# laclouis5/StructureDetector

Hardware: NVIDIA B200
Metric: decoded images/s (higher is better)
Workload: dtype f32

## Files before the change

### structuredetector_b200/csrc/common.cuh

```cuda
#pragma once

#include <cuda.h>
#include <cuda_bf16.h>
#include <cuda_fp16.h>
#include <cuda_runtime.h>
#include <math_constants.h>
#include <stdint.h>
#include <stdlib.h>

#include "sdnet_decode.h"

namespace {

typedef unsigned long long u64;
typedef unsigned int u32;

constexpr int kThreads = 256;
constexpr int kWarps = kThreads / 32;
constexpr int kPanelW = 128;
constexpr int kBins = 128;
constexpr float kBinLo = -16.0f;
constexpr float kBinScale = 4.0f;
constexpr int kFineBins = 512;
constexpr float kFineScale = 16.0f;
// ... 52 lines not shown
    const float s = __half2float(__float2half_rn(1.0f / (1.0f + expf(-x))));
    return __half2float(__float2half_rn(fminf(fmaxf(s, kClampLo), kClampHi)));
  }
  static __device__ __forceinline__ float to_float(__half v) { return __half2float(v); }
};

template <>
struct Num<SDNET_DTYPE_BF16> {
  typedef __nv_bfloat16 In;
  static constexpr float kNear = 0.1f, kHi = 2.0f, kLo = -13.0f;
  static constexpr float kNear2 = 0.6f, kHi2 = 4.0f;
  static __device__ __forceinline__ float act(float x) {
    const float s = __bfloat162float(__float2bfloat16_rn(1.0f / (1.0f + expf(-x))));
    return __bfloat162float(__float2bfloat16_rn(fminf(fmaxf(s, kClampLo), kClampHi)));
  }
  static __device__ __forceinline__ float to_float(__nv_bfloat16 v) { return __bfloat162float(v); }
};

template <int DT>
__device__ __forceinline__ float ld_in(const void* base, long long idx) {
  return Num<DT>::to_float(__ldg(static_cast<const typename Num<DT>::In*>(base) + idx));
}

__device__ __forceinline__ float max3(float a, float b, float c) { return fmaxf(fmaxf(a, b), c); }

__device__ __forceinline__ void pdl_launch_dependents() { asm volatile("griddepcontrol.launch_dependents;" ::: "memory"); }
__device__ __forceinline__ void pdl_wait() { asm volatile("griddepcontrol.wait;" ::: "memory"); }

__device__ __forceinline__ float comp(const float4& v, int j) {
  return j == 0 ? v.x : (j == 1 ? v.y : (j == 2 ? v.z : v.w));
}

__device__ __forceinline__ u32 smem_u32(const void* p) { return (u32)__cvta_generic_to_shared(p); }
__device__ __forceinline__ void cp_async4_if(u32 dst, const void* src, bool pred) {
  asm volatile("{\n\t.reg .pred p;\n\tsetp.ne.b32 p, %2, 0;\n\t@p cp.async.ca.shared.global [%0], [%1], 4;\n\t}"
               ::"r"(dst), "l"(src), "r"((int)pred));
}
__device__ __forceinline__ void cp_async_commit() { asm volatile("cp.async.commit_group;" ::: "memory"); }
template <int N>
__device__ __forceinline__ void cp_async_wait() { asm volatile("cp.async.wait_group %0;" ::"n"(N) : "memory"); }
__device__ __forceinline__ float4 lds128(u32 addr) {
  float4 v;
  asm volatile("ld.shared.v4.f32 {%0, %1, %2, %3}, [%4];" : "=f"(v.x), "=f"(v.y), "=f"(v.z), "=f"(v.w) : "r"(addr));
  return v;
}
__device__ __forceinline__ float2 lds64(u32 addr) {
  float2 v;
  asm volatile("ld.shared.v2.f32 {%0, %1}, [%2];" : "=f"(v.x), "=f"(v.y) : "r"(addr));
  return v;
}
__device__ __forceinline__ void sts128(u32 addr, float a) {
  asm volatile("st.shared.v4.f32 [%0], {%1, %1, %1, %1};" ::"r"(addr), "f"(a) : "memory");
}
__device__ __forceinline__ void sts64(u32 addr, float a) {
  asm volatile("st.shared.v2.f32 [%0], {%1, %1};" ::"r"(addr), "f"(a) : "memory");
}

__device__ __forceinline__ void mbar_init(u32 bar, u32 count) {
  asm volatile("mbarrier.init.shared::cta.b64 [%0], %1;" ::"r"(bar), "r"(count) : "memory");
}
__device__ __forceinline__ void mbar_fence_init() { asm volatile("fence.mbarrier_init.release.cluster;" ::: "memory"); }
__device__ __forceinline__ void mbar_arrive_expect_tx(u32 bar, u32 bytes) {
  asm volatile("mbarrier.arrive.expect_tx.shared::cta.b64 _, [%0], %1;" ::"r"(bar), "r"(bytes) : "memory");
}
#ifndef SDNET_X_WAIT_NS
#define SDNET_X_WAIT_NS 1000
#endif
__device__ __forceinline__ void mbar_wait(u32 bar, u32 parity) {
#if SDNET_X_WAIT_NS > 0
  asm volatile(
      "{\n\t.reg .pred p;\n"
      "WAIT_LOOP:\n\t"
      "mbarrier.try_wait.parity.shared::cta.b64 p, [%0], %1, %2;\n\t"
      "@!p bra WAIT_LOOP;\n\t}"
      ::"r"(bar), "r"(parity), "r"((u32)SDNET_X_WAIT_NS) : "memory");
#else
  asm volatile(
      "{\n\t.reg .pred p;\n"
      "WAIT_LOOP:\n\t"
      "mbarrier.try_wait.parity.shared::cta.b64 p, [%0], %1;\n\t"
      "@!p bra WAIT_LOOP;\n\t}"
      ::"r"(bar), "r"(parity) : "memory");
#endif
}
__device__ __forceinline__ void fence_proxy_async() { asm volatile("fence.proxy.async.shared::cta;" ::: "memory"); }

}
```

### structuredetector_b200/csrc/floors.cuh

```cuda
#pragma once

namespace {

#ifndef SDNET_X_BUF
#define SDNET_X_BUF 64
#endif
constexpr int kBuf = SDNET_X_BUF;
#ifndef SDNET_X_GRATE
#define SDNET_X_GRATE 0
#endif
#ifndef SDNET_X_LRATE
#define SDNET_X_LRATE 0
#endif
constexpr int kGRate = SDNET_X_GRATE, kLRate = SDNET_X_LRATE;
constexpr int kGDiv = kGRate ? kGRate : 1, kLDiv = kLRate ? kLRate : 1;

__device__ __forceinline__ int logit_bin(float x) {
  int bin = __float2int_rd((x - kBinLo) * kBinScale);
  bin = max(0, min(kBins - 1, bin));
  if (bin > 0 && x < kBinLo + (float)bin * (1.0f / kBinScale)) --bin;
  return bin;
}

__device__ __forceinline__ int ord_of(float x) {
  const int b = __float_as_int(x);
  return b ^ ((b >> 31) & 0x7fffffff);
}
__device__ __forceinline__ float ord_to_float(int o) { return __int_as_float(o ^ ((o >> 31) & 0x7fffffff)); }

__device__ __forceinline__ int floor_bin_of(const uint4 c, int lane, int K) {
  const u32 s = c.x + c.y + c.z + c.w;
  u32 suf = s;
#pragma unroll
  for (int d = 1; d < 32; d <<= 1) {
    u32 t = __shfl_down_sync(0xffffffffu, suf, d);
    if (lane + d < 32) suf += t;
  }
  const u32 mask = __ballot_sync(0xffffffffu, suf >= (u32)K);
  if (mask == 0) return -1;
  const int L = 31 - __clz(mask);
  int b = 0;
  if (lane == L) {
    u32 above = suf - s;
    if (above + c.w >= (u32)K) b = 4 * L + 3;
    else if (above + c.w + c.z >= (u32)K) b = 4 * L + 2;
    else if (above + c.w + c.z + c.y >= (u32)K) b = 4 * L + 1;
    else b = 4 * L;
  }
  return __shfl_sync(0xffffffffu, b, L);
}

__device__ __forceinline__ float local_floor(const u32* hist, const int* minx, int lane, int K) {
  const int b = floor_bin_of(*reinterpret_cast<const uint4*>(hist + 4 * lane), lane, K);
  if (b < 0) return -CUDART_INF_F;
  return ord_to_float(minx[b]);
}

__device__ __forceinline__ int fine_bin(float x) {
  static_assert(kBinLo == -16.0f && kFineScale == 16.0f, "bin arithmetic below");
  return max(0, min(kFineBins - 1, __float2int_rd(fminf(fmaxf(x * kFineScale, -4096.0f), 4096.0f)) + 256));
// ... 16 lines not shown
  uint4 v[kFinePerLane / 4];
#pragma unroll
  for (int q = 0; q < kFinePerLane / 4; ++q) v[q] = load_bins<kShared>(mine + 4 * q);
  u32 s = 0;
#pragma unroll
  for (int q = 0; q < kFinePerLane / 4; ++q) s += v[q].x + v[q].y + v[q].z + v[q].w;
  u32 suf = s;
#pragma unroll
  for (int d = 1; d < 32; d <<= 1) {
    u32 t = __shfl_down_sync(0xffffffffu, suf, d);
    if (lane + d < 32) suf += t;
  }
  const u32 mask = __ballot_sync(0xffffffffu, suf >= (u32)K);
  if (mask == 0) return -1;
  const int L = 31 - __clz(mask);
  int b = kFinePerLane * L;
  if (lane == L) {
    u32 above = suf - s;
    bool found = false;
#pragma unroll
    for (int q = kFinePerLane / 4 - 1; q >= 0; --q) {
      const u32 c4[4] = {v[q].x, v[q].y, v[q].z, v[q].w};
#pragma unroll
      for (int e = 3; e >= 0; --e) {
        if (!found) {
          if (above + c4[e] >= (u32)K) { b = kFinePerLane * L + 4 * q + e; found = true; }
          else above += c4[e];
        }
      }
    }
  }
  return __shfl_sync(0xffffffffu, b, L);
}

template <int DT = SDNET_DTYPE_F32>
__device__ __forceinline__ float shared_floor(int fbin, float xscale) {
  const bool pre = xscale != 1.0f;
  if (fbin <= 0) return pre ? 0.0f : -CUDART_INF_F;
  const float edge = kBinLo + (float)fbin * (1.0f / kFineScale);
  if (pre) return fmaxf(edge / xscale, 0.0f);
  if (edge < Num<DT>::kLo || edge > Num<DT>::kHi2) return -CUDART_INF_F;
  return edge - (edge <= Num<DT>::kHi ? Num<DT>::kNear : Num<DT>::kNear2);
}

struct SharedFloors {
  u32* ghist;
  int* gfloor;
};

struct UnitState {
  float floorx;
  u32 emitted;
  int nbuf;
};

template <int DT = SDNET_DTYPE_F32, bool kFlushCountsFine = true>
__device__ __forceinline__ void flush_candidates(UnitState& st, const u64* buf, u32* hist, int* minx,
                                                 const SharedFloors& sf, int* count_ptr, u64* __restrict__ list,
                                                 int cap, int K, int lane, bool pre, float xscale, float satx) {
  const int n = st.nbuf;
  int base = 0;
  if (lane == 0) base = atomicAdd(count_ptr, n);
  base = __shfl_sync(0xffffffffu, base, 0);
#pragma unroll
  for (int half = 0; half < kBuf / 32; ++half) {
    const int i = half * 32 + lane;
    if (half * 32 < n) {
      const bool valid = i < n;
      const u64 rec = valid ? buf[i] : 0ull;
      const float x = __uint_as_float((u32)(rec >> 32));
      u32 key;
      if (pre) {
        const u32 bits = __float_as_uint(x);
        key = (bits & 0x80000000u) ? ~bits : (bits | 0x80000000u);
      } else {
        key = __float_as_uint(Num<DT>::act(x));
      }
      if (valid) {
        if (base + i < cap) list[base + i] = ((u64)key << 32) | (u32)rec;
        const float xe = fminf(fmaxf(x * xscale, -satx), satx);
        const int bin = logit_bin(xe);
        atomicAdd(&hist[bin], 1u);
        atomicMin(&minx[bin], ord_of(xe));
        if (kFlushCountsFine && sf.ghist) atomicAdd(&sf.ghist[fine_bin(xe)], 1u);
      }
    }
  }
  const u32 before = st.emitted;
  st.emitted += n;
  st.nbuf = 0;
  __syncwarp();
  if (st.emitted >= (u32)K && (kLRate == 0 || before < (u32)K || before / kLDiv != st.emitted / kLDiv))
    st.floorx = fmaxf(st.floorx, local_floor(hist, minx, lane, K) / xscale);
  if (sf.ghist && base + n >= K && (kGRate == 0 || base < K || base / kGDiv != (base + n) / kGDiv)) {
    const int gb = floor_bin_fine<false>(sf.ghist, lane, K);
    if (gb > 0) {
      if (lane == 0) atomicMax(sf.gfloor, gb);
      st.floorx = fmaxf(st.floorx, shared_floor<DT>(gb, xscale));
    }
  }
  if (st.floorx >= satx) st.floorx = CUDART_INF_F;
}


}
```

### structuredetector_b200/csrc/peaks_tile.cuh

```cuda
#pragma once

namespace {

constexpr int kGroupRows = 4;
constexpr int kTileCols = kPanelW + 8;
constexpr int kTilePitchB = kTileCols * 4;
constexpr int kTileBytes = kGroupRows * kTilePitchB;
#ifndef SDNET_X_WARPS
#define SDNET_X_WARPS 4
#endif
constexpr int kTileWarps = SDNET_X_WARPS;
#ifndef SDNET_X_CTAS
#define SDNET_X_CTAS (24 / SDNET_X_WARPS)
#endif
constexpr int kTileMinCtas = SDNET_X_CTAS;
constexpr int kMinChunkGroups = 8;
#ifndef SDNET_X_NG
#define SDNET_X_NG 3
#endif
constexpr int kTileNG = SDNET_X_NG;
#ifndef SDNET_X_FLUSH_AT
#define SDNET_X_FLUSH_AT 16
#endif
constexpr int kWork = 128;
constexpr int kFlushAt = SDNET_X_FLUSH_AT;
__host__ __device__ constexpr int tile_slot_bytes(int S) { return S == 1 ? kTileBytes : 2304; }
__host__ __device__ constexpr int tile_smem_per_warp(int S) {
  return ((kTileNG * tile_slot_bytes(S) + 32 + kBins * 8 + kBuf * 8 + kWork) + 127) / 128 * 128;
}
__host__ __device__ constexpr int tile_smem(int S) { return kTileWarps * tile_smem_per_warp(S); }
constexpr int kOddBoxOff = 1152;
constexpr int kOddShiftB = 8;

template <int DT>
struct TileGeom {
  static constexpr int kPx = DT == SDNET_DTYPE_F32 ? 4 : 8;
  static constexpr int kEsz = 16 / kPx;
  static constexpr int kPanel = 32 * kPx;
  static constexpr int kCols = kPanel + 2 * kPx;
};
static_assert(TileGeom<SDNET_DTYPE_F32>::kCols * 4 == kTilePitchB && TileGeom<SDNET_DTYPE_F16>::kCols * 2 == kTilePitchB, "ring row pitch");

__device__ __forceinline__ void tma_tile_4d(u32 dst, const CUtensorMap* map, int x, int y, int c, int b, u32 bar) {
  asm volatile(
      "cp.async.bulk.tensor.4d.shared::cluster.global.tile.mbarrier::complete_tx::bytes [%0], [%1, {%2, %3, %4, %5}], [%6];"
      ::"r"(dst), "l"(map), "r"(x), "r"(y), "r"(c), "r"(b), "r"(bar) : "memory");
}
__device__ __forceinline__ uint4 lds64x2(u32 addr) {
  uint4 v;
  asm volatile("ld.shared.v2.u32 {%0, %1}, [%2];" : "=r"(v.x), "=r"(v.y) : "r"(addr));
  asm volatile("ld.shared.v2.u32 {%0, %1}, [%2];" : "=r"(v.z), "=r"(v.w) : "r"(addr + 8));
  return v;
}
__device__ __forceinline__ uint4 lds128u(u32 addr) {
  uint4 v;
  asm volatile("ld.shared.v4.u32 {%0, %1, %2, %3}, [%4];" : "=r"(v.x), "=r"(v.y), "=r"(v.z), "=r"(v.w) : "r"(addr));
  return v;
}

template <int DT>
struct TileMax;
template <>
struct TileMax<SDNET_DTYPE_F32> {
  static __device__ __forceinline__ float word(const uint4& a) {
    return fmaxf(fmaxf(__uint_as_float(a.x), __uint_as_float(a.y)), fmaxf(__uint_as_float(a.z), __uint_as_float(a.w)));
  }
  static __device__ __forceinline__ float group(const uint4& a, const uint4& b, const uint4& c, const uint4& d) {
    return fmaxf(fmaxf(word(a), word(b)), fmaxf(word(c), word(d)));
  }
  static __device__ __forceinline__ float elem(u32 addr) {
    float v;
    asm volatile("ld.shared.f32 %0, [%1];" : "=f"(v) : "r"(addr));
    return v;
  }
  static __device__ __forceinline__ u32 raw(u32 addr) { return __float_as_uint(elem(addr)); }
  static __device__ __forceinline__ u32 rmax(u32 a, u32 b) { return __float_as_uint(fmaxf(__uint_as_float(a), __uint_as_float(b))); }
  static __device__ __forceinline__ float rfloat(u32 r) { return __uint_as_float(r); }
};
template <>
struct TileMax<SDNET_DTYPE_F16> {
  static __device__ __forceinline__ __half2 h2(u32 v) { return *reinterpret_cast<const __half2*>(&v); }
  static __device__ __forceinline__ __half2 word2(const uint4& a) { return __hmax2(__hmax2(h2(a.x), h2(a.y)), __hmax2(h2(a.z), h2(a.w))); }
  static __device__ __forceinline__ float fold(__half2 m) { return __half2float(__hmax(__low2half(m), __high2half(m))); }
// ... 84 lines not shown
    for (int d = 0; d <= 2 * R; ++d) {
      u32 rr = row0 + i + d;
      if (rr >= kRingRows) rr -= kRingRows;
      roff[d] = S == 1 ? rr * kTilePitchB : __shfl_sync(0xffffffffu, row_tab, (int)rr);
    }
    const float x = TileMax<DT>::elem(col_addr + R * kEsz + roff[R]);
    bool keep = slot < nslots && x > floorx;
#if SDNET_X_QUICK
    if (!pre) {
      const u32 ctr = col_addr + R * kEsz;
      const float m4 = fmaxf(fmaxf(TileMax<DT>::elem(ctr + roff[R - 1]), TileMax<DT>::elem(ctr + roff[R + 1])),
                             fmaxf(TileMax<DT>::elem(ctr - kEsz + roff[R]), TileMax<DT>::elem(ctr + kEsz + roff[R])));
      if (x < m4 - kNearTie2 && x <= kHiZone2 - 1.0f && x >= kLoZone) keep = false;
    }
#endif
    if (keep && !pre) {
      u32 hr[2 * R + 1];
#pragma unroll
      for (int d = 0; d <= 2 * R; ++d) {
        const u32 a = col_addr + roff[d];
        u32 v[2 * R + 1];
#pragma unroll
        for (int q = 0; q <= 2 * R; ++q) v[q] = TileMax<DT>::raw(a + kEsz * q);
        hr[d] = v[0];
#pragma unroll
        for (int q = 1; q <= 2 * R; ++q) hr[d] = TileMax<DT>::rmax(hr[d], v[q]);
      }
#pragma unroll
      for (int d = 1; d <= 2 * R; ++d) hr[0] = TileMax<DT>::rmax(hr[0], hr[d]);
      const float h = fmaxf(x, TileMax<DT>::rfloat(hr[0]));
      if (x != h) {
        const bool amb = (x >= h - kNearTie) || (h > kHiZone && x >= h - kNearTie2) ||
                         (h > kHiZone2 && x > kHiZone2 - 1.0f) || (h < kLoZone);
        keep = amb && Num<DT>::act(x) == Num<DT>::act(h);
      }
    }
    const u32 m = __ballot_sync(0xffffffffu, keep);
    if (m) {
      if (st.nbuf + __popc(m) > kBuf) {
        __syncwarp();
        flush_candidates<DT, !SDNET_X_EARLYHIST>(st, buf, hist, minx, sf, count_ptr, list, cap, K, lane, pre, xscale, satx);
      }
      if (keep) {
        buf[st.nbuf + __popc(m & ((1u << lane) - 1u))] = ((u64)__float_as_uint(x) << 32) | (idx0 + i * (u32)W + colp);
#if SDNET_X_EARLYHIST
        atomicAdd(&sf.ghist[fine_bin(fminf(fmaxf(x * xscale, -satx), satx))], 1u);
#endif
      }
      st.nbuf += __popc(m);
    }
  }
}

#ifndef SDNET_X_DENSE
#define SDNET_X_DENSE 16
#endif
constexpr int kDenseLanes = SDNET_X_DENSE;


template <int R>
__device__ __forceinline__ u32 dense_keep_mask_f32(int rows_here, u32 ring_s, u32 ring_own, u32 row0, float floorx, bool pre, int lane) {
  constexpr int DT = SDNET_DTYPE_F32;
  constexpr float kNearTie = Num<DT>::kNear, kHiZone = Num<DT>::kHi, kLoZone = Num<DT>::kLo;
  constexpr u32 kRingRows = kTileNG * kGroupRows;
  const u32 halo_a = ring_s + (lane == 31 ? 33u * 16u : 0u);
  u32 km = 0;
#pragma unroll
  for (int i = 0; i < kGroupRows; ++i) {
    if (i < rows_here) {
      float4 v, xc;
      float2 ev;
#pragma unroll
      for (int d = 0; d <= 2 * R; ++d) {
        u32 rr = row0 + i + d;
        if (rr >= kRingRows) rr -= kRingRows;
        const float4 a = lds128(ring_own + rr * kTilePitchB);
        const float4 w = lds128(halo_a + rr * kTilePitchB);
        const float2 e = lane == 31 ? make_float2(w.x, w.y) : make_float2(w.z, w.w);
        if (d == 0) {
          v = a;
          ev = e;
        } else {
          v.x = fmaxf(v.x, a.x); v.y = fmaxf(v.y, a.y); v.z = fmaxf(v.z, a.z); v.w = fmaxf(v.w, a.w);
          ev.x = fmaxf(ev.x, e.x); ev.y = fmaxf(ev.y, e.y);
        }
        if (d == R) xc = a;
      }
      float l2 = __shfl_up_sync(0xffffffffu, v.z, 1), l3 = __shfl_up_sync(0xffffffffu, v.w, 1);
      float r0 = __shfl_down_sync(0xffffffffu, v.x, 1), r1 = __shfl_down_sync(0xffffffffu, v.y, 1);
      if (lane == 0) { l2 = ev.x; l3 = ev.y; }
      if (lane == 31) { r0 = ev.x; r1 = ev.y; }
      float4 h;
      if (R == 2) {
        h.x = max3(max3(l2, l3, v.x), v.y, v.z);
        h.y = max3(max3(l3, v.x, v.y), v.z, v.w);
        h.z = max3(max3(v.x, v.y, v.z), v.w, r0);
        h.w = max3(max3(v.y, v.z, v.w), r0, r1);
      } else {
        h.x = max3(l3, v.x, v.y);
        h.y = max3(v.x, v.y, v.z);
        h.z = max3(v.y, v.z, v.w);
        h.w = max3(v.z, v.w, r0);
      }
#pragma unroll
      for (int c = 0; c < 4; ++c) {
        const float x = comp(xc, c), hh = comp(h, c);
// ... 51 lines not shown

template <int DT>
__device__ __forceinline__ void tile_fix_edges(u32 slot_s, int x0, int W, int lane) {
  constexpr int kPx = TileGeom<DT>::kPx;
  constexpr u32 kNinf2 = DT == SDNET_DTYPE_F16 ? 0xFC00FC00u : (DT == SDNET_DTYPE_BF16 ? 0xFF80FF80u : 0xFF800000u);
  if (x0 < 0) {
    if (lane < 2) {
      const u32 a = slot_s + kOddBoxOff + lane * kTilePitchB;
      asm volatile("st.shared.v4.u32 [%0], {%1, %1, %1, %1};" ::"r"(a), "r"(kNinf2) : "memory");
      asm volatile("st.shared.v2.u32 [%0], {%1, %1};" ::"r"(a + 16), "r"(kNinf2) : "memory");
    }
  }
  if (x0 + TileGeom<DT>::kCols > W) {
#pragma unroll
    for (int k = 0; k < 2; ++k) {
      const int w = k == 0 ? lane + 1 : 33;
      if (k == 1 && lane != 31) break;
      const int first = x0 + kPx * w;
      const u32 a = slot_s + 16 * w;
      if (first >= W) {
        asm volatile("st.shared.v4.u32 [%0], {%1, %1, %1, %1};" ::"r"(a), "r"(kNinf2) : "memory");
        asm volatile("st.shared.v4.u32 [%0], {%1, %1, %1, %1};" ::"r"(a + kTilePitchB), "r"(kNinf2) : "memory");
      } else if (first + kPx / 2 >= W) {
        asm volatile("st.shared.v2.u32 [%0], {%1, %1};" ::"r"(a + 8), "r"(kNinf2) : "memory");
        asm volatile("st.shared.v2.u32 [%0], {%1, %1};" ::"r"(a + 8 + kTilePitchB), "r"(kNinf2) : "memory");
      }
    }
  }
}

#if SDNET_X_TRACE
__device__ unsigned long long g_tile_trace[8192 * 4];
__device__ __forceinline__ unsigned long long trace_now() {
  unsigned long long t;
  asm volatile("mov.u64 %0, %%globaltimer;" : "=l"(t));
  return t;
}
#endif

template <int R, int DT, int S>
__global__ void __launch_bounds__(kTileWarps * 32, kTileMinCtas)
sdnet_peaks_tile_kernel(const __grid_constant__ PeaksParams p, const __grid_constant__ CUtensorMap tm_anchor,
                        const __grid_constant__ CUtensorMap tm_part) {
  extern __shared__ __align__(128) unsigned char smem_raw[];
  constexpr int NG = kTileNG;
  constexpr u32 kRingRows = NG * kGroupRows;
  constexpr int kPx = TileGeom<DT>::kPx, kPanel = TileGeom<DT>::kPanel;
  static_assert(NG >= 3 && kRingRows <= 32, "a group reads two slots; ring-row offsets are looked up by lane");
  static_assert(S == 1 || (R == 2 && DT != SDNET_DTYPE_F32), "row pairs: tiles must start on an even row");
  pdl_launch_dependents();
  const int lane = threadIdx.x & 31;
  const int warp = threadIdx.x >> 5;
  constexpr u32 kSlotB = tile_slot_bytes(S);
  unsigned char* wbase = smem_raw + (size_t)warp * tile_smem_per_warp(S);
  const u32 ring_s = smem_u32(wbase);
  const u32 bars_s = ring_s + NG * kSlotB;
  u32* hist = reinterpret_cast<u32*>(wbase + NG * kSlotB + 32);
  int* minx = reinterpret_cast<int*>(hist + kBins);
  u64* buf = reinterpret_cast<u64*>(minx + kBins);
  unsigned char* work = reinterpret_cast<unsigned char*>(buf + kBuf);
  const u32 lt = (1u << lane) - 1u;
  const bool pre = p.pre_activated != 0;
  const float xscale = pre ? kPreScale : 1.0f;
  const float satx = pre ? CUDART_INF_F : kSatX;
  const int C = p.M + p.N;
  const int H = p.H, W = p.W;
  const u32 ring_own = ring_s + (u32)(16 + 16 * lane);
  const u32 row_tab = ring_row_off<S>((u32)lane % kRingRows);

  if (lane == 0) {
    for (int i = 0; i < NG; ++i) mbar_init(bars_s + 8 * i, 1);
    mbar_fence_init();
  }
  __syncwarp();

  u32 cur_slot = 0, cur_par = 0;
  auto step_pos = [&](u32& slot, u32& par) {
    if (++slot == (u32)NG) { slot = 0; par ^= 1u; }
  };
#if SDNET_X_TRACE
  const unsigned long long tr_start = trace_now();
  unsigned long long tr_first = 0, tr_groups = 0, tr_units = 0;
#endif
  for (;;) {
    u32 unit = 0;
    if (lane == 0) unit = atomicAdd(p.sched, 1u);
    unit = __shfl_sync(0xffffffffu, unit, 0);
    if (unit >= (u32)p.units) break;
#if SDNET_X_TRACE
    ++tr_units;
#endif
    u32 pos, pos_end;
    if (unit < (u32)p.tier1_units) {
      pos = unit * (u32)p.groups_per_col;
      pos_end = pos + (u32)p.groups_per_col;
    } else {
      pos = (u32)p.tier1_units * (u32)p.groups_per_col + (unit - (u32)p.tier1_units) * (u32)p.chunk_groups;
      pos_end = min(p.total_groups, pos + (u32)p.chunk_groups);
    }
    while (pos < pos_end) {
    const u32 column = pos / (u32)p.groups_per_col;
    const int g_first = (int)(pos - column * (u32)p.groups_per_col);
    const int g_last = min(p.groups_per_col, g_first + (int)(pos_end - pos));
    pos += (u32)(g_last - g_first);
    const int panel = (int)(column % (u32)p.panels), plane_id = (int)(column / (u32)p.panels);
    const int r_begin = g_first * kGroupRows, r_end = min(H, g_last * kGroupRows);
    const int b = plane_id / C, c = plane_id % C;
    const bool is_anchor = c < p.M;
    const CUtensorMap* tmap = is_anchor ? &tm_anchor : &tm_part;
    const int csel = is_anchor ? c : c - p.M;
    const int K = is_anchor ? p.K : p.P;
    const int x0 = panel * kPanel - kPx;
    const int xc = DT == SDNET_DTYPE_F32 ? x0 : x0 >> 1;
    const bool edge = S == 2 && (x0 < 0 || x0 + TileGeom<DT>::kCols > W);
    const int nrows = r_end - r_begin;
    const int groups = (nrows + 2 * R + kGroupRows - 1) / kGroupRows;
    const int groups_out = (nrows + kGroupRows - 1) / kGroupRows;
    u64* __restrict__ list = p.lists + (size_t)plane_id * p.cap;
    int* count_ptr = p.counts + plane_id;
    int* gfloor_ptr = p.gfloor + plane_id;
    SharedFloors sf;
    sf.ghist = p.ghist + (size_t)plane_id * kFineBins;
    sf.gfloor = gfloor_ptr;

    UnitState st;
    st.floorx = shared_floor<DT>(__ldcg(gfloor_ptr), xscale);
    st.emitted = 0;
    st.nbuf = 0;
    __syncwarp();
    *reinterpret_cast<uint4*>(hist + 4 * lane) = make_uint4(0, 0, 0, 0);
    *reinterpret_cast<int4*>(minx + 4 * lane) = make_int4(0x7fffffff, 0x7fffffff, 0x7fffffff, 0x7fffffff);
    __syncwarp();

    auto issue = [&](u32 s, int y) {
      mbar_arrive_expect_tx(bars_s + 8 * s, kTileBytes);
      if (S == 1) {
        tma_tile_4d(ring_s + s * kSlotB, tmap, xc, y, csel, b, bars_s + 8 * s);
      } else {
        tma_tile_4d(ring_s + s * kSlotB, tmap, xc, y >> 1, csel, b, bars_s + 8 * s);
        tma_tile_4d(ring_s + s * kSlotB + kOddBoxOff, tmap, xc + p.odd_x - kOddShiftB / 4, y >> 1, csel, b, bars_s + 8 * s);
      }
    };
    auto wait_tile = [&](u32 slot, u32 par) {
      mbar_wait(bars_s + 8 * slot, par);
      if (edge) {
        tile_fix_edges<DT>(ring_s + slot * kSlotB, x0, W, lane);
        __syncwarp();
      }
    };
    int y_next = r_begin - R;
    if (lane == 0) {
      const int first = min(NG, groups);
      u32 sl = cur_slot;
      for (int k = 0; k < first; ++k) {
        issue(sl, y_next + kGroupRows * k);
        if (++sl == (u32)NG) sl = 0;
      }
    }
    y_next += kGroupRows * NG;
    int gfloor_seen = 0;
    constexpr int poll_mask = 3;
    u32 idx0 = (u32)(r_begin * W + panel * kPanel);
    wait_tile(cur_slot, cur_par);
#if SDNET_X_TRACE
    if (!tr_first) tr_first = trace_now();
    tr_groups += (unsigned long long)groups_out;
#endif
    for (int g = 0; g < groups_out; ++g, idx0 += (u32)(kGroupRows * W)) {
      u32 nxt_slot = cur_slot, nxt_par = cur_par;
      step_pos(nxt_slot, nxt_par);
      if (R == 2 || g + 1 < groups) wait_tile(nxt_slot, nxt_par);
#if SDNET_X_WARMPOLL
      if (gfloor_seen <= 0 && g > 0) {
        gfloor_seen = __ldcg(gfloor_ptr);
        st.floorx = fmaxf(st.floorx, shared_floor<DT>(gfloor_seen, xscale));
      } else
#endif
      if ((g & poll_mask) == 0) {
        st.floorx = fmaxf(st.floorx, shared_floor<DT>(gfloor_seen, xscale));
        asm volatile("ld.global.cg.s32 %0, [%1];" : "=r"(gfloor_seen) : "l"(gfloor_ptr) : "memory");
      }
      const u32 row0 = cur_slot * kGroupRows;
      uint4 c0, c1, c2, c3;
      if (R == 2) {
        const u32 a01 = ring_own + cur_slot * kSlotB, a23 = ring_own + nxt_slot * kSlotB;
        if (S == 1) {
          c0 = lds128u(a01 + 2 * kTilePitchB); c1 = lds128u(a01 + 3 * kTilePitchB);
          c2 = lds128u(a23); c3 = lds128u(a23 + kTilePitchB);
        } else {
          c0 = lds128u(a01 + kTilePitchB); c1 = lds64x2(a01 + kOddBoxOff + kOddShiftB + kTilePitchB);
          c2 = lds128u(a23); c3 = lds64x2(a23 + kOddBoxOff + kOddShiftB);
        }
      } else {
        const u32 a012 = ring_own + (row0 + 1) * kTilePitchB, a3 = ring_own + nxt_slot * kGroupRows * kTilePitchB;
        c0 = lds128u(a012); c1 = lds128u(a012 + kTilePitchB); c2 = lds128u(a012 + 2 * kTilePitchB); c3 = lds128u(a3);
      }
      const u32 hot = __ballot_sync(0xffffffffu, TileMax<DT>::group(c0, c1, c2, c3) > st.floorx);
      if (hot) {
        const int nhot = __popc(hot), rows_here = nrows - g * kGroupRows;
        const float floorx = st.floorx;
        bool settled = false;
        if (DT == SDNET_DTYPE_F32 && S == 1 && kDenseLanes > 0 && nhot >= kDenseLanes)
          settled = settle_dense_f32<R>(st, rows_here, ring_s, ring_own, row0, floorx, idx0, W, pre, buf, hist, minx, sf, count_ptr,
                                        list, p.cap, K, lane, xscale, satx);
        if (!settled) {
          int nent = 0;
#pragma unroll
          for (int i = 0; i < kGroupRows; ++i) {
            const uint4 ci = i == 0 ? c0 : (i == 1 ? c1 : (i == 2 ? c2 : c3));
            const bool mine = TileMax<DT>::word(ci) > floorx && i < rows_here;
            const u32 bm = __ballot_sync(0xffffffffu, mine);
            if (mine) work[nent + __popc(bm & lt)] = (unsigned char)((i << 5) | lane);
            nent += __popc(bm);
          }
          __syncwarp();
          settle_entries<R, DT, S>(st, work, nent, ring_s, row0, row_tab, floorx, idx0, W, pre, buf, hist, minx, sf, count_ptr, list,
                                   p.cap, K, lane, xscale, satx);
        }
        if (st.nbuf >= kFlushAt || (SDNET_X_EARLYFLUSH && st.nbuf > 0 && gfloor_seen <= 0)) {
          __syncwarp();
          flush_candidates<DT, !SDNET_X_EARLYHIST>(st, buf, hist, minx, sf, count_ptr, list, p.cap, K, lane, pre, xscale, satx);
        }
      }
      __syncwarp();
      if (lane == 0 && g + NG < groups) {
        if (edge) fence_proxy_async();
        issue(cur_slot, y_next);
      }
      y_next += kGroupRows;
      cur_slot = nxt_slot;
      cur_par = nxt_par;
    }
    for (int k = groups_out; k < groups; ++k) step_pos(cur_slot, cur_par);
    if (st.nbuf) {
      __syncwarp();
      flush_candidates<DT, !SDNET_X_EARLYHIST>(st, buf, hist, minx, sf, count_ptr, list, p.cap, K, lane, pre, xscale, satx);
    }
    }
  }
#if SDNET_X_TRACE
  if (lane == 0) {
    const u32 w = blockIdx.x * kTileWarps + warp;
    if (w < 8192) {
      g_tile_trace[4 * w + 0] = tr_start; g_tile_trace[4 * w + 1] = tr_first; g_tile_trace[4 * w + 2] = trace_now();
      g_tile_trace[4 * w + 3] = (tr_groups << 32) | tr_units;
    }
  }
#endif
}


}
```

### structuredetector_b200/csrc/sdnet_decode.cu

```cuda
#include <atomic>
#include <mutex>

#include "common.cuh"
#include "floors.cuh"
#include "peaks_warp.cuh"
#include "peaks_tile.cuh"
#include "exact_select.cuh"
#include "tail.cuh"
#include "match.cuh"
#include "sweep.cuh"
#include "suppress.cuh"

namespace {

struct Workspace {
  size_t off_counts, off_flags, off_sched, off_gfloor, off_ghist, off_lists, total;
  int cap;
};

inline size_t align_up(size_t v, size_t a) { return (v + a - 1) / a * a; }

Workspace plan_workspace(int B, int M, int N, int H, int W, int K, int P) {
  Workspace ws;
  const size_t planes = (size_t)B * (M + N);
// ... 174 lines not shown
  int n = 0;
  *err = cudaOccupancyMaxActiveBlocksPerMultiprocessor(&n, kern, kTileWarps * 32, smem);
  if (*err != cudaSuccess) return 0;
  per_sm = n < 1 ? 1 : n;
  return per_sm;
}

struct PeaksPlan {
  int path, tile_s;
  TileKernel tile_kern;
  int smem, ctas, ctas_per_sm, sms;
  CUtensorMap tm_anchor, tm_part;
};

bool plan_tile_line(PeaksParams& pp, long long planes, long long resident, int chunk_override, int* ctas, long long max_ctas) {
  const long long G = (pp.H + kGroupRows - 1) / kGroupRows;
  const long long columns = planes * pp.panels;
  if (columns * G >= (1ll << 31)) return false;
  const long long tier1 = (columns / resident) * resident;
  const long long rest = (columns - tier1) * G;
  long long chunk = (rest + resident - 1) / resident;
  if (chunk < kMinChunkGroups) chunk = kMinChunkGroups;
  if (chunk_override > 0) chunk = chunk_override;
  if (chunk > G) chunk = G;
  pp.tier1_units = (int)tier1;
  pp.groups_per_col = (int)G;
  pp.chunk_groups = (int)chunk;
  pp.total_groups = (u32)(columns * G);
  pp.units = (int)(tier1 + (rest + chunk - 1) / chunk);
  long long n = ((long long)pp.units + kTileWarps - 1) / kTileWarps;
  if (n > max_ctas) n = max_ctas;
  *ctas = (int)n;
  return true;
}

cudaError_t plan_peaks(const SdnetDecodeParams* p, PeaksParams& pp, PeaksPlan& pl) {
  const int C = p->M + p->N;
  const long long planes = (long long)p->B * C;
  pl.sms = device_sm_count();
  pl.tile_s = 0;
  pl.path = select_peaks_path(p, &pl.tm_anchor, &pl.tm_part, &pl.tile_s);
  const bool use_tile = pl.path == SDNET_PATH_TILE || pl.path == SDNET_PATH_TILE_ROW_PAIRS;
  const bool is_f32 = p->dtype == SDNET_DTYPE_F32;
  pp.odd_x = (int)(p->anchor_hm.stride_h / (is_f32 ? 1 : 2));
  pp.tier1_units = 0;
  pp.groups_per_col = 0;
  pp.chunk_groups = 0;
  pp.total_groups = 0;
  pp.strips = 1;
  pp.rows_per_strip = p->H;
  if (use_tile) {
    pl.tile_kern = tile_kernel_for(p->radius, p->dtype, pl.tile_s);
    const int panel_cols = is_f32 ? TileGeom<SDNET_DTYPE_F32>::kPanel : TileGeom<SDNET_DTYPE_F16>::kPanel;
    pl.smem = tile_smem(pl.tile_s);
    cudaError_t err = cudaSuccess;
    pl.ctas_per_sm = tile_ctas_per_sm(pl.tile_kern, p->dtype, pl.tile_s, p->radius, pl.smem, &err);
    if (pl.ctas_per_sm <= 0) return err != cudaSuccess ? err : cudaErrorUnknown;
    static const int occ_cap = [] {
      const char* e = getenv("SDNET_PEAKS_OCC");
      return e ? atoi(e) : 0;
    }();
    if (occ_cap > 0 && occ_cap < pl.ctas_per_sm) pl.ctas_per_sm = occ_cap;
    pp.panels = (p->W + panel_cols - 1) / panel_cols;
    static const int chunk_override = [] {
      const char* e = getenv("SDNET_CHUNK_GROUPS");
      return e ? atoi(e) : 0;
    }();
    pp.H = p->H;
    if (!plan_tile_line(pp, planes, (long long)pl.sms * pl.ctas_per_sm * kTileWarps, chunk_override, &pl.ctas,
                        (long long)pl.sms * pl.ctas_per_sm))
      return cudaErrorInvalidValue;
  } else {
    pl.tile_kern = nullptr;
    pl.smem = kPeaksSmem;
    pl.ctas_per_sm = kPeaksCtasPerSm;
    pp.panels = (p->W + kPanelW - 1) / kPanelW;
    const long long resident = (long long)pl.sms * kPeaksCtasPerSm * kWarps;
    const long long units1 = planes * pp.panels;
    int strips = (int)((4 * resident + units1 - 1) / units1);
    const int max_strips = (p->H + 31) / 32;
    if (strips > max_strips) strips = max_strips;
    if (strips < 1) strips = 1;
    pp.rows_per_strip = (p->H + strips - 1) / strips;
    pp.strips = (p->H + pp.rows_per_strip - 1) / pp.rows_per_strip;
    if (planes * pp.strips * pp.panels >= (1ll << 31)) return cudaErrorInvalidValue;
    pp.units = (int)(planes * pp.strips * pp.panels);
    long long ctas = ((long long)pp.units + kWarps - 1) / kWarps;
    if (ctas > (long long)pl.sms * kPeaksCtasPerSm) ctas = (long long)pl.sms * kPeaksCtasPerSm;
    pl.ctas = (int)ctas;
  }
  return cudaSuccess;
}

int launch_decode(const SdnetDecodeParams* p, cudaStream_t stream, cudaEvent_t* marks = nullptr) {
  const Workspace ws = plan_workspace(p->B, p->M, p->N, p->H, p->W, p->K, p->P);
  char* base = static_cast<char*>(p->workspace);
  const int C = p->M + p->N;
  const size_t planes = (size_t)p->B * C;
  const int sms = device_sm_count();

  PeaksParams pp;
  pp.anchor = to_view(p->anchor_hm);
  pp.part = to_view(p->part_hm);
  pp.B = p->B; pp.M = p->M; pp.N = p->N; pp.H = p->H; pp.W = p->W; pp.K = p->K; pp.P = p->P;
  pp.cap = ws.cap;
  pp.pre_activated = (p->flags & SDNET_FLAG_PRE_ACTIVATED) ? 1 : 0;
  pp.lists = reinterpret_cast<u64*>(base + ws.off_lists);
// ... 147 lines not shown
  if (p->struct_size != sizeof(SdnetObjectMatchParams)) return SDNET_E_STRUCT;
  if (!p->anchor_out || !p->part_out || !p->assign || !p->image_scale || !p->n_gt_objects || !p->n_gt_parts || !p->cls_group ||
      !p->csi_stats || !p->csi_acc || !p->classif_stats || !p->classif_acc || !p->pred_parts ||
      (p->max_gt_objects > 0 && !p->gt_objects) || (p->max_gt_parts > 0 && (!p->gt_parts || !p->gt_part_owner)))
    return SDNET_E_NULL;
  if (p->B <= 0 || p->M <= 0 || p->N <= 0 || p->K <= 0 || p->P <= 0 || p->K > SDNET_MAX_TOPK || p->P > SDNET_MAX_TOPK ||
      p->M + p->N > SDNET_MAX_CHANNELS || p->max_gt_objects < 0 || p->max_gt_parts < 0 || p->max_gt_objects > SDNET_MAX_GT ||
      p->max_gt_parts > SDNET_MAX_GT)
    return SDNET_E_SHAPE;
  const size_t smem = match_objects_smem_bytes(p->max_gt_objects, p->max_gt_parts, p->K, p->P, p->M);
  cudaError_t err = cudaFuncSetAttribute(sdnet_match_objects_kernel, cudaFuncAttributeMaxDynamicSharedMemorySize, (int)smem);
  if (err != cudaSuccess) return (int)err;
  sdnet_match_objects_kernel<<<dim3((unsigned)p->B), dim3(kMatchThreads), smem, static_cast<cudaStream_t>(stream)>>>(*p);
  return (int)cudaGetLastError();
}

int sdnet_sweep_launch(const SdnetSweepParams* p, void* stream) {
  if (!p) return SDNET_E_NULL;
  if (p->struct_size != sizeof(SdnetSweepParams)) return SDNET_E_STRUCT;
  const bool objects = (p->flags & SDNET_SWEEP_OBJECTS) != 0;
  if (!p->conf || !p->conf_group || !p->anchor_out || !p->part_out || !p->image_scale || !p->n_gt_objects ||
      !p->n_gt_parts || !p->anchor_stats || !p->part_stats || !p->anchor_acc || !p->part_acc ||
      (p->max_gt_objects > 0 && !p->gt_objects) || (p->max_gt_parts > 0 && !p->gt_parts) ||
      (p->G >= 1 && !p->dist_abs_grid))
    return SDNET_E_NULL;
  if (objects && (!p->cls_group || !p->csi_stats || !p->csi_acc || !p->classif_stats || !p->classif_acc ||
                  !p->pred_parts || (p->max_gt_parts > 0 && !p->gt_part_owner)))
    return SDNET_E_NULL;
  if (p->B <= 0 || p->M <= 0 || p->N <= 0 || p->K <= 0 || p->P <= 0 || p->K > SDNET_MAX_TOPK || p->P > SDNET_MAX_TOPK ||
      p->M + p->N > SDNET_MAX_CHANNELS || p->T < 1 || p->T > SDNET_MAX_THRESHOLDS || p->max_gt_objects < 0 ||
      p->max_gt_parts < 0 || p->max_gt_objects > SDNET_MAX_GT || p->max_gt_parts > SDNET_MAX_GT ||
      p->G < 0 || p->G > SDNET_MAX_GATES || (long long)p->B * p->T * (p->G > 1 ? p->G : 1) > 0x7fffffffll)
    return SDNET_E_SHAPE;
  const size_t smem = sweep_smem_bytes(*p);
  cudaError_t err = cudaFuncSetAttribute(sdnet_sweep_kernel, cudaFuncAttributeMaxDynamicSharedMemorySize, (int)smem);
  if (err != cudaSuccess) return (int)err;
  sdnet_sweep_kernel<<<dim3((unsigned)(p->B * p->T)), dim3(kMatchThreads), smem, static_cast<cudaStream_t>(stream)>>>(*p);
  return (int)cudaGetLastError();
}

int sdnet_decode_peaks_path(const SdnetDecodeParams* params) {
  const int rc = validate(params);
  if (rc != 0) return rc;
  CUtensorMap a, b;
  int tile_s = 0;
  return select_peaks_path(params, &a, &b, &tile_s);
}

#if SDNET_X_TRACE
int sdnet_debug_trace(unsigned long long* out, int n_warps) {
  return (int)cudaMemcpyFromSymbol(out, g_tile_trace, sizeof(unsigned long long) * 4 * (size_t)n_warps);
}
#endif

int sdnet_decode_schedule(const SdnetDecodeParams* params, SdnetSchedule* out) {
  const int rc = validate(params);
  if (rc != 0) return rc;
  if (!out) return SDNET_E_NULL;
  if (out->struct_size != sizeof(SdnetSchedule)) return SDNET_E_STRUCT;
  PeaksParams pp;
  PeaksPlan pl;
  const cudaError_t err = plan_peaks(params, pp, pl);
  if (err != cudaSuccess) return (int)err;
  out->path = pl.path;
  out->units = pp.units;
  out->tier1_units = pp.tier1_units;
  out->chunk_units = pl.tile_kern ? pp.units - pp.tier1_units : 0;
  out->chunk_groups = pp.chunk_groups;
  out->groups_per_column = pp.groups_per_col;
  out->panels = pp.panels;
  out->strips = pp.strips;
  out->rows_per_strip = pp.rows_per_strip;
  out->ctas = pl.ctas;
  out->warps_per_cta = pl.tile_kern ? kTileWarps : kWarps;
  out->ctas_per_sm = pl.ctas_per_sm;
  out->sms = pl.sms;
  out->list_capacity = plan_workspace(params->B, params->M, params->N, params->H, params->W, params->K, params->P).cap;
  return 0;
}

int sdnet_decode_launch(const SdnetDecodeParams* params, void* stream) {
  const int rc = validate(params);
  if (rc) return rc;
  return launch_decode(params, static_cast<cudaStream_t>(stream));
}

int sdnet_decode_launch_timed(const SdnetDecodeParams* params, void* stream_v, float* kernel_ms) {
  const int rc = validate(params);
  if (rc) return rc;
  if (!kernel_ms) return SDNET_E_NULL;
  cudaStream_t stream = static_cast<cudaStream_t>(stream_v);
  cudaEvent_t marks[4];
  for (int i = 0; i < 4; ++i) {
    cudaError_t e = cudaEventCreate(&marks[i]);
    if (e != cudaSuccess) return (int)e;
  }
  int out = launch_decode(params, stream, marks);
  if (out == 0) {
    cudaError_t e = cudaEventSynchronize(marks[3]);
    if (e != cudaSuccess) out = (int)e;
    for (int i = 0; i < 3 && out == 0; ++i) {
      e = cudaEventElapsedTime(&kernel_ms[i], marks[i], marks[i + 1]);
      if (e != cudaSuccess) out = (int)e;
    }
  }
  for (int i = 0; i < 4; ++i) cudaEventDestroy(marks[i]);
// ... 110 lines not shown
```

Baseline: 1.376 million.

## Park sparse hot words into a side buffer and settle them in batched drains

For the f32 radius-2 tile path, groups with only a few above-floor words no longer run the list settle pass right away. Each such word's 5x8 neighbourhood is copied into a per-warp parking area in shared memory, up to seven entries. When the area would overflow, when a dense group arrives, or when the unit ends, all parked entries are settled together in one warp pass at four lanes per word, so sparse groups stop wasting most lanes. This adds shared memory per warp, which can lower occupancy, adds copy traffic, and settles later against a floor that may have risen since parking. Optional stats counters are also added but are compiled out by default.

```diff
diff --git a/structuredetector_b200/csrc/common.cuh b/structuredetector_b200/csrc/common.cuh
--- a/structuredetector_b200/csrc/common.cuh
+++ b/structuredetector_b200/csrc/common.cuh
@@ -128,6 +128,12 @@
 __device__ __forceinline__ void sts128(u32 addr, float a) {
   asm volatile("st.shared.v4.f32 [%0], {%1, %1, %1, %1};" ::"r"(addr), "f"(a) : "memory");
 }
+__device__ __forceinline__ u32 lds_u32(u32 addr) {
+  u32 v;
+  asm volatile("ld.shared.u32 %0, [%1];" : "=r"(v) : "r"(addr) : "memory");
+  return v;
+}
+__device__ __forceinline__ void sts_u32(u32 addr, u32 v) { asm volatile("st.shared.u32 [%0], %1;" ::"r"(addr), "r"(v) : "memory"); }
 __device__ __forceinline__ void sts64(u32 addr, float a) {
   asm volatile("st.shared.v2.f32 [%0], {%1, %1};" ::"r"(addr), "f"(a) : "memory");
 }
diff --git a/structuredetector_b200/csrc/floors.cuh b/structuredetector_b200/csrc/floors.cuh
--- a/structuredetector_b200/csrc/floors.cuh
+++ b/structuredetector_b200/csrc/floors.cuh
@@ -6,6 +6,9 @@
 #define SDNET_X_BUF 64
 #endif
 constexpr int kBuf = SDNET_X_BUF;
+#ifndef SDNET_X_STATS
+#define SDNET_X_STATS 0
+#endif
 #ifndef SDNET_X_GRATE
 #define SDNET_X_GRATE 0
 #endif
@@ -128,6 +131,9 @@
   float floorx;
   u32 emitted;
   int nbuf;
+#if SDNET_X_STATS
+  u32 flushes;
+#endif
 };
 
 template <int DT = SDNET_DTYPE_F32, bool kFlushCountsFine = true>
@@ -164,6 +170,9 @@
   }
   const u32 before = st.emitted;
   st.emitted += n;
+#if SDNET_X_STATS
+  ++st.flushes;
+#endif
   st.nbuf = 0;
   __syncwarp();
   if (st.emitted >= (u32)K && (kLRate == 0 || before < (u32)K || before / kLDiv != st.emitted / kLDiv))
diff --git a/structuredetector_b200/csrc/peaks_tile.cuh b/structuredetector_b200/csrc/peaks_tile.cuh
--- a/structuredetector_b200/csrc/peaks_tile.cuh
+++ b/structuredetector_b200/csrc/peaks_tile.cuh
@@ -24,11 +24,21 @@
 #endif
 constexpr int kWork = 128;
 constexpr int kFlushAt = SDNET_X_FLUSH_AT;
+#ifndef SDNET_X_PARK
+#define SDNET_X_PARK 7
+#endif
+constexpr int kParkN = SDNET_X_PARK;
+constexpr int kParkRowB = 32;
+constexpr int kParkRegionB = 5 * kParkRowB;
+static_assert(kParkN >= 0 && kParkN <= 8, "a drain is one pass: four lanes per parked word");
 __host__ __device__ constexpr int tile_slot_bytes(int S) { return S == 1 ? kTileBytes : 2304; }
-__host__ __device__ constexpr int tile_smem_per_warp(int S) {
-  return ((kTileNG * tile_slot_bytes(S) + 32 + kBins * 8 + kBuf * 8 + kWork) + 127) / 128 * 128;
-}
-__host__ __device__ constexpr int tile_smem(int S) { return kTileWarps * tile_smem_per_warp(S); }
+__host__ __device__ constexpr int tile_park_entries(int R, int DT, int S) {
+  return R == 2 && DT == SDNET_DTYPE_F32 && S == 1 ? kParkN : 0;
+}
+__host__ __device__ constexpr int tile_smem_per_warp(int S, int npark) {
+  return ((kTileNG * tile_slot_bytes(S) + 32 + kBins * 8 + kBuf * 8 + kWork + npark * (kParkRegionB + 4)) + 127) / 128 * 128;
+}
+__host__ __device__ constexpr int tile_smem(int S, int npark) { return kTileWarps * tile_smem_per_warp(S, npark); }
 constexpr int kOddBoxOff = 1152;
 constexpr int kOddShiftB = 8;
 
@@ -219,6 +229,77 @@
   }
 }
 
+template <int DT, int kPk>
+__device__ __forceinline__ void settle_parked(UnitState& st, int npark, u32 park_s, u64* buf, u32* hist,
+                                              int* minx, const SharedFloors& sf, int* count_ptr, u64* __restrict__ list, int cap,
+                                              int K, int lane, float xscale, float satx) {
+  static_assert(DT == SDNET_DTYPE_F32, "parked regions hold fp32 words");
+  constexpr int R = 2;
+  constexpr float kNearTie = Num<DT>::kNear, kHiZone = Num<DT>::kHi, kLoZone = Num<DT>::kLo, kNearTie2 = Num<DT>::kNear2,
+                  kHiZone2 = Num<DT>::kHi2;
+  const bool live = (lane >> 2) < npark;
+  const int e = live ? lane >> 2 : 0;
+  const u32 a = park_s + (u32)e * kParkRegionB + 4u * (u32)(lane & 3);
+  const u32 ctr = a + R * kParkRowB + R * 4;
+  const float floorx = st.floorx;
+  const float x = TileMax<DT>::elem(ctr);
+  bool keep = live && x > floorx;
+#if SDNET_X_QUICK
+  const float m4 = fmaxf(fmaxf(TileMax<DT>::elem(ctr - kParkRowB), TileMax<DT>::elem(ctr + kParkRowB)),
+                         fmaxf(TileMax<DT>::elem(ctr - 4), TileMax<DT>::elem(ctr + 4)));
+  if (x < m4 - kNearTie2 && x <= kHiZone2 - 1.0f && x >= kLoZone) keep = false;
+#endif
+  if (keep) {
+    float hr[2 * R + 1];
+#pragma unroll
+    for (int d = 0; d <= 2 * R; ++d) {
+      float v[2 * R + 1];
+#pragma unroll
+      for (int q = 0; q <= 2 * R; ++q) v[q] = TileMax<DT>::elem(a + d * kParkRowB + 4 * q);
+      hr[d] = v[0];
+#pragma unroll
+      for (int q = 1; q <= 2 * R; ++q) hr[d] = fmaxf(hr[d], v[q]);
+    }
+#pragma unroll
+    for (int d = 1; d <= 2 * R; ++d) hr[0] = fmaxf(hr[0], hr[d]);
+    const float h = fmaxf(x, hr[0]);
+    if (x != h) {
+      const bool amb = (x >= h - kNearTie) || (h > kHiZone && x >= h - kNearTie2) ||
+                       (h > kHiZone2 && x > kHiZone2 - 1.0f) || (h < kLoZone);
+      keep = amb && Num<DT>::act(x) == Num<DT>::act(h);
+    }
+  }
+  const u32 m = __ballot_sync(0xffffffffu, keep);
+  if (m) {
+    if (st.nbuf + __popc(m) > kBuf) {
+      __syncwarp();
+      flush_candidates<DT, !SDNET_X_EARLYHIST>(st, buf, hist, minx, sf, count_ptr, list, cap, K, lane, false, xscale, satx);
+    }
+    if (keep) {
+      u32 idx;
+      asm volatile("ld.shared.u32 %0, [%1];" : "=r"(idx) : "r"(park_s + kPk * kParkRegionB + 4u * (u32)e));
+      buf[st.nbuf + __popc(m & ((1u << lane) - 1u))] = ((u64)__float_as_uint(x) << 32) | (idx + (u32)(lane & 3));
+#if SDNET_X_EARLYHIST
+      atomicAdd(&sf.ghist[fine_bin(fminf(fmaxf(x * xscale, -satx), satx))], 1u);
+#endif
+    }
+    st.nbuf += __popc(m);
+  }
+  __syncwarp();
+}
+
+#if SDNET_X_STATS
+enum PeaksStat {
+  kStFast, kStDense, kStList, kStParked,
+  kStWords1, kStWords2, kStWords4, kStWords8,
+  kStPasses, kStPassLanes, kStDrains, kStDrainLanes,
+  kStFlushes, kStRecords,
+  kStCycles,
+  kStN = kStCycles + 15
+};
+__device__ unsigned long long g_peaks_stats[kStN];
+#endif
+
 #ifndef SDNET_X_DENSE
 #define SDNET_X_DENSE 16
 #endif
@@ -376,13 +457,21 @@
   const int lane = threadIdx.x & 31;
   const int warp = threadIdx.x >> 5;
   constexpr u32 kSlotB = tile_slot_bytes(S);
-  unsigned char* wbase = smem_raw + (size_t)warp * tile_smem_per_warp(S);
+  constexpr int kPk = tile_park_entries(R, DT, S);
+  unsigned char* wbase = smem_raw + (size_t)warp * tile_smem_per_warp(S, kPk);
   const u32 ring_s = smem_u32(wbase);
   const u32 bars_s = ring_s + NG * kSlotB;
   u32* hist = reinterpret_cast<u32*>(wbase + NG * kSlotB + 32);
   int* minx = reinterpret_cast<int*>(hist + kBins);
   u64* buf = reinterpret_cast<u64*>(minx + kBins);
   unsigned char* work = reinterpret_cast<unsigned char*>(buf + kBuf);
+  auto park_addr = [&](u32 off) {
+    u32 a;
+    asm volatile("add.u32 %0, %1, %2;" : "=r"(a) : "r"(ring_s), "r"(off));
+    return a;
+  };
+  constexpr u32 kParkOff = NG * kSlotB + 32 + kBins * 8 + kBuf * 8 + kWork, kNParkOff = NG * kSlotB + 8 * NG;
+  static_assert(8 * NG + 4 <= 32, "the barrier block holds NG mbarriers and the park count");
   const u32 lt = (1u << lane) - 1u;
   const bool pre = p.pre_activated != 0;
   const float xscale = pre ? kPreScale : 1.0f;
@@ -405,6 +494,10 @@
 #if SDNET_X_TRACE
   const unsigned long long tr_start = trace_now();
   unsigned long long tr_first = 0, tr_groups = 0, tr_units = 0;
+#endif
+#if SDNET_X_STATS
+  unsigned long long sx[kStN];
+  for (int k = 0; k < kStN; ++k) sx[k] = 0;
 #endif
   for (;;) {
     u32 unit = 0;
@@ -451,6 +544,10 @@
     st.floorx = shared_floor<DT>(__ldcg(gfloor_ptr), xscale);
     st.emitted = 0;
     st.nbuf = 0;
+#if SDNET_X_STATS
+    st.flushes = 0;
+#endif
+    if (kPk > 0 && lane == 0) sts_u32(park_addr(kNParkOff), 0u);
     __syncwarp();
     *reinterpret_cast<uint4*>(hist + 4 * lane) = make_uint4(0, 0, 0, 0);
     *reinterpret_cast<int4*>(minx + 4 * lane) = make_int4(0x7fffffff, 0x7fffffff, 0x7fffffff, 0x7fffffff);
@@ -504,6 +601,9 @@
         st.floorx = fmaxf(st.floorx, shared_floor<DT>(gfloor_seen, xscale));
         asm volatile("ld.global.cg.s32 %0, [%1];" : "=r"(gfloor_seen) : "l"(gfloor_ptr) : "memory");
       }
+#if SDNET_X_STATS
+      const unsigned long long st_t0 = clock64();
+#endif
       const u32 row0 = cur_slot * kGroupRows;
       uint4 c0, c1, c2, c3;
       if (R == 2) {
@@ -520,32 +620,104 @@
         c0 = lds128u(a012); c1 = lds128u(a012 + kTilePitchB); c2 = lds128u(a012 + 2 * kTilePitchB); c3 = lds128u(a3);
       }
       const u32 hot = __ballot_sync(0xffffffffu, TileMax<DT>::group(c0, c1, c2, c3) > st.floorx);
+#if SDNET_X_STATS
+      const int st_pos = g_first + g < 8 ? 0 : (g_first + g < 32 ? 1 : 2);
+      int st_path = kStFast;
+      unsigned long long st_drain = 0;
+#endif
       if (hot) {
         const int nhot = __popc(hot), rows_here = nrows - g * kGroupRows;
         const float floorx = st.floorx;
-        bool settled = false;
-        if (DT == SDNET_DTYPE_F32 && S == 1 && kDenseLanes > 0 && nhot >= kDenseLanes)
-          settled = settle_dense_f32<R>(st, rows_here, ring_s, ring_own, row0, floorx, idx0, W, pre, buf, hist, minx, sf, count_ptr,
-                                        list, p.cap, K, lane, xscale, satx);
-        if (!settled) {
-          int nent = 0;
+        auto list_words = [&]() {
+          int n = 0;
 #pragma unroll
           for (int i = 0; i < kGroupRows; ++i) {
             const uint4 ci = i == 0 ? c0 : (i == 1 ? c1 : (i == 2 ? c2 : c3));
             const bool mine = TileMax<DT>::word(ci) > floorx && i < rows_here;
             const u32 bm = __ballot_sync(0xffffffffu, mine);
-            if (mine) work[nent + __popc(bm & lt)] = (unsigned char)((i << 5) | lane);
-            nent += __popc(bm);
+            if (mine) work[n + __popc(bm & lt)] = (unsigned char)((i << 5) | lane);
+            n += __popc(bm);
           }
           __syncwarp();
+          return n;
+        };
+        bool settled = false;
+        int nent = -1;
+        if constexpr (kPk > 0) {
+          const bool sparse = !pre && nhot < kDenseLanes;
+          if (sparse) nent = list_words();
+          const bool park = sparse && nent <= kPk;
+          int npark = (int)lds_u32(park_addr(kNParkOff));
+          if (npark > 0 && (!park || nent > kPk - npark)) {
+#if SDNET_X_STATS
+            st_drain = clock64();
+            sx[kStDrains] += 1;
+            sx[kStDrainLanes] += 4 * npark;
+#endif
+            settle_parked<DT, kPk>(st, npark, park_addr(kParkOff), buf, hist, minx, sf, count_ptr, list, p.cap, K, lane, xscale, satx);
+            npark = 0;
+            if (!park && lane == 0) sts_u32(park_addr(kNParkOff), 0u);
+#if SDNET_X_STATS
+            st_drain = clock64() - st_drain;
+            sx[kStCycles + 3 * 4 + st_pos] += st_drain;
+#endif
+          }
+          if (park) {
+            if (lane < nent) {
+              const u32 ent = work[lane], i = ent >> 5, wl = ent & 31u;
+              const u32 src = ring_s + 8u + 16u * wl, dst = park_addr(kParkOff + (u32)(npark + lane) * kParkRegionB);
+#pragma unroll
+              for (int d = 0; d <= 2 * R; ++d) {
+                u32 rr = row0 + i + d;
+                if (rr >= kRingRows) rr -= kRingRows;
+                const u32 a = src + rr * kTilePitchB;
+                const float2 l = lds64(a);
+                const float4 w = lds128(a + 8);
+                const float2 r = lds64(a + 24);
+                const u32 o = dst + d * kParkRowB;
+                asm volatile("st.shared.v4.f32 [%0], {%1, %2, %3, %4};" ::"r"(o), "f"(l.x), "f"(l.y), "f"(w.x), "f"(w.y) : "memory");
+                asm volatile("st.shared.v4.f32 [%0], {%1, %2, %3, %4};" ::"r"(o + 16), "f"(w.z), "f"(w.w), "f"(r.x), "f"(r.y) : "memory");
+              }
+              asm volatile("st.shared.u32 [%0], %1;" ::"r"(park_addr(kParkOff + kPk * kParkRegionB + 4u * (u32)(npark + lane))),
+                           "r"(idx0 + i * (u32)W + 4u * wl) : "memory");
+            }
+            npark += nent;
+            if (lane == 0) sts_u32(park_addr(kNParkOff), (u32)npark);
+            settled = true;
+#if SDNET_X_STATS
+            st_path = kStParked;
+#endif
+          }
+        }
+        if (!settled && DT == SDNET_DTYPE_F32 && S == 1 && kDenseLanes > 0 && nhot >= kDenseLanes) {
+          settled = settle_dense_f32<R>(st, rows_here, ring_s, ring_own, row0, floorx, idx0, W, pre, buf, hist, minx, sf, count_ptr,
+                                        list, p.cap, K, lane, xscale, satx);
+#if SDNET_X_STATS
+          if (settled) st_path = kStDense;
+#endif
+        }
+        if (!settled) {
+          if (nent < 0) nent = list_words();
           settle_entries<R, DT, S>(st, work, nent, ring_s, row0, row_tab, floorx, idx0, W, pre, buf, hist, minx, sf, count_ptr, list,
                                    p.cap, K, lane, xscale, satx);
+#if SDNET_X_STATS
+          st_path = kStList;
+          sx[kStPasses] += (4 * nent + 31) / 32;
+          sx[kStPassLanes] += 4 * nent;
+#endif
         }
+#if SDNET_X_STATS
+        if (nent > 0) sx[nent == 1 ? kStWords1 : (nent < 4 ? kStWords2 : (nent < 8 ? kStWords4 : kStWords8))] += 1;
+#endif
         if (st.nbuf >= kFlushAt || (SDNET_X_EARLYFLUSH && st.nbuf > 0 && gfloor_seen <= 0)) {
           __syncwarp();
           flush_candidates<DT, !SDNET_X_EARLYHIST>(st, buf, hist, minx, sf, count_ptr, list, p.cap, K, lane, pre, xscale, satx);
         }
       }
+#if SDNET_X_STATS
+      sx[st_path] += 1;
+      sx[kStCycles + 3 * st_path + st_pos] += clock64() - st_t0 - st_drain;
+#endif
       __syncwarp();
       if (lane == 0 && g + NG < groups) {
         if (edge) fence_proxy_async();
@@ -556,10 +728,28 @@
       cur_par = nxt_par;
     }
     for (int k = groups_out; k < groups; ++k) step_pos(cur_slot, cur_par);
+    if constexpr (kPk > 0) {
+      const int npark = (int)lds_u32(park_addr(kNParkOff));
+      if (npark > 0) {
+#if SDNET_X_STATS
+        const unsigned long long t0 = clock64();
+        sx[kStDrains] += 1;
+        sx[kStDrainLanes] += 4 * npark;
+#endif
+        settle_parked<DT, kPk>(st, npark, park_addr(kParkOff), buf, hist, minx, sf, count_ptr, list, p.cap, K, lane, xscale, satx);
+#if SDNET_X_STATS
+        sx[kStCycles + 3 * 4 + 2] += clock64() - t0;
+#endif
+      }
+    }
     if (st.nbuf) {
       __syncwarp();
       flush_candidates<DT, !SDNET_X_EARLYHIST>(st, buf, hist, minx, sf, count_ptr, list, p.cap, K, lane, pre, xscale, satx);
     }
+#if SDNET_X_STATS
+    sx[kStFlushes] += st.flushes;
+    sx[kStRecords] += st.emitted;
+#endif
     }
   }
 #if SDNET_X_TRACE
@@ -571,7 +761,12 @@
     }
   }
 #endif
-}
-
-
-}
+#if SDNET_X_STATS
+  if (lane == 0)
+    for (int k = 0; k < kStN; ++k)
+      if (sx[k]) atomicAdd(&g_peaks_stats[k], sx[k]);
+#endif
+}
+
+
+}
diff --git a/structuredetector_b200/csrc/sdnet_decode.cu b/structuredetector_b200/csrc/sdnet_decode.cu
--- a/structuredetector_b200/csrc/sdnet_decode.cu
+++ b/structuredetector_b200/csrc/sdnet_decode.cu
@@ -250,7 +250,7 @@
   if (use_tile) {
     pl.tile_kern = tile_kernel_for(p->radius, p->dtype, pl.tile_s);
     const int panel_cols = is_f32 ? TileGeom<SDNET_DTYPE_F32>::kPanel : TileGeom<SDNET_DTYPE_F16>::kPanel;
-    pl.smem = tile_smem(pl.tile_s);
+    pl.smem = tile_smem(pl.tile_s, tile_park_entries(p->radius, p->dtype, pl.tile_s));
     cudaError_t err = cudaSuccess;
     pl.ctas_per_sm = tile_ctas_per_sm(pl.tile_kern, p->dtype, pl.tile_s, p->radius, pl.smem, &err);
     if (pl.ctas_per_sm <= 0) return err != cudaSuccess ? err : cudaErrorUnknown;
@@ -504,6 +504,17 @@
   return (int)cudaMemcpyFromSymbol(out, g_tile_trace, sizeof(unsigned long long) * 4 * (size_t)n_warps);
 }
 #endif
+#if SDNET_X_STATS
+int sdnet_debug_stats(unsigned long long* out, int n) {
+  if (!out) return SDNET_E_NULL;
+  if (n != kStN) return SDNET_E_SHAPE;
+  cudaError_t e = cudaDeviceSynchronize();
+  if (e == cudaSuccess) e = cudaMemcpyFromSymbol(out, g_peaks_stats, sizeof(unsigned long long) * kStN);
+  static const unsigned long long zero[kStN] = {};
+  if (e == cudaSuccess) e = cudaMemcpyToSymbol(g_peaks_stats, zero, sizeof(zero));
+  return (int)e;
+}
+#endif
 
 int sdnet_decode_schedule(const SdnetDecodeParams* params, SdnetSchedule* out) {
   const int rc = validate(params);
```

Measured after the change: 1.226 million (median of 6 runs). -10.9%, worse.
